# nyu-systems/Grendel-GS

Measured on AMD Instinct MI355X. Metric: training iters/sec (fwd+bwd), higher is better.
Workload: dtype f32

## Files before the change

grendel-gs_amd/csrc/binning_persist.h:

```cpp
#pragma once

namespace {

constexpr int TT_SHIFT = 20;
constexpr uint32_t TT_MASK = (1u << TT_SHIFT) - 1u;
constexpr uint32_t GB_ABORT = 0x80000000u;
constexpr int GB_FAN = 32;
constexpr int GB_LEAF_STRIDE = 32;
constexpr uint32_t PAIRS_ABORTED = 0xFFFFFFFFu;

struct GridSync {
    uint32_t *leaf;
    uint32_t *root;
    uint32_t *flags;
};
__host__ __device__ inline size_t grid_sync_words(int G) {
    return (size_t)(2 * ((G + GB_FAN - 1) / GB_FAN) + 1) * GB_LEAF_STRIDE;
}

__device__ __forceinline__ bool grid_barrier_try_abort(const GridSync gs, uint32_t complete) {
    uint32_t r = __hip_atomic_load(gs.root, __ATOMIC_RELAXED, __HIP_MEMORY_SCOPE_AGENT);
    while (true) {
        if (r & GB_ABORT) return true;
        if (r == complete) return false;
// ... 232 lines not shown
    out.ys = (uint32_t)miny | ((uint32_t)maxy << 16);
    out.mask = ~0ull;
    if (!cull || w * h > 64) {
        if (dxy) {
            atomicAdd(&dxy[0][minx], h);
            atomicAdd(&dxy[0][maxx], -h);
            atomicAdd(&dxy[1][miny], w);
            atomicAdd(&dxy[1][maxy], -w);
            atomicAdd(&dxy[2][miny], 1);
            atomicAdd(&dxy[2][maxy], -1);
        }
        return (uint32_t)(w * h);
    }
    const unsigned long long mask = gsr_tile_mask(xy, co, minx, miny, maxx, maxy);
    out.mask = mask;
    if (dxy) {
        const unsigned long long rowm = gsr_full_mask(w);
        int prev_cnt = 0, run_a0 = 0, run_len = 0, run_mult = 0;
        for (int r = 0; r < h; r++) {
            unsigned long long bits = (mask >> (r * w)) & rowm;
            const int cnt = __popcll(bits);
            if (cnt != prev_cnt) atomicAdd(&dxy[1][miny + r], cnt - prev_cnt);
            prev_cnt = cnt;
            while (bits) {
                const int a0 = __ffsll((long long)bits) - 1;
                const unsigned long long rest = ~(bits >> a0);
                const int len = rest ? __ffsll((long long)rest) - 1 : 64 - a0;
                if (run_mult && a0 == run_a0 && len == run_len) {
                    run_mult++;
                } else {
                    if (run_mult) {
                        atomicAdd(&dxy[0][minx + run_a0], run_mult);
                        atomicAdd(&dxy[0][minx + run_a0 + run_len], -run_mult);
                    }
                    run_a0 = a0; run_len = len; run_mult = 1;
                }
                bits &= ~(gsr_full_mask(len) << a0);
            }
        }
        if (run_mult) {
            atomicAdd(&dxy[0][minx + run_a0], run_mult);
            atomicAdd(&dxy[0][minx + run_a0 + run_len], -run_mult);
        }
        if (prev_cnt) atomicAdd(&dxy[1][maxy], -prev_cnt);
    }
    return (uint32_t)__popcll(mask);
}

template <int ITEMS, int THREADS>
struct PersistSmem {
    uint16_t wtab[THREADS / 64][RADIX_DIGITS];
    uint32_t gbase[RADIX_DIGITS];
    unsigned long long scan64[THREADS / 64];
    uint32_t scan_tmp[THREADS / 64];
    uint32_t flag;
    uint32_t skey[ITEMS * THREADS], sval[ITEMS * THREADS];
};

template <int ITEMS, int THREADS>
__device__ __forceinline__ void clear_wtab(PersistSmem<ITEMS, THREADS> &sm) {
    uint32_t *p = reinterpret_cast<uint32_t *>(&sm.wtab[0][0]);
    for (int i = threadIdx.x; i < (THREADS / 64) * RADIX_DIGITS / 2; i += THREADS) p[i] = 0u;
}

struct ByteDigit {
    int shift;
    uint32_t mask;
    __device__ __forceinline__ uint32_t operator()(uint32_t k) const { return (k >> shift) & mask; }
};
constexpr int BK_BINS = 4096, BK_BIN_BITS = 12;
constexpr uint32_t BK_TAIL = 255u;
struct BucketDigit {
    const uint8_t *map;
    uint32_t kmin;
    int sh;
    __device__ __forceinline__ uint32_t operator()(uint32_t k) const {
        return k == 0xFFFFFFFFu ? BK_TAIL : (uint32_t)map[(k - kmin) >> sh];
    }
};

template <int ITEMS, int THREADS, class DG>
__device__ __forceinline__ void count_wave_digits(PersistSmem<ITEMS, THREADS> &sm, const uint32_t (&key)[ITEMS],
                                                  long long wbase, long long n, const DG digit) {
    const int lane = threadIdx.x & 63, wave = threadIdx.x >> 6;
#pragma unroll
    for (int r = 0; r < ITEMS; r++) {
        if (wbase + r * 64 + lane < n) {
            const uint32_t dg = digit(key[r]);
            atomicAdd(reinterpret_cast<uint32_t *>(sm.wtab[wave]) + (dg >> 1), 1u << (16 * (dg & 1u)));
        }
    }
}
template <int ITEMS, int THREADS>
__device__ __forceinline__ void count_wave_digits(PersistSmem<ITEMS, THREADS> &sm, const uint32_t (&key)[ITEMS],
                                                  long long wbase, long long n, int shift, uint32_t mask) {
    count_wave_digits(sm, key, wbase, n, ByteDigit{shift, mask});
}

template <int ITEMS, int THREADS, class DG>
__device__ __forceinline__ void scatter_rank(PersistSmem<ITEMS, THREADS> &sm, const uint32_t (&key)[ITEMS],
                                             const uint32_t (&val)[ITEMS], long long tbase, long long n, const DG digit,
                                             int nbits, uint32_t &tot_out, uint32_t &run_out) {
    constexpr int WAVES = THREADS / 64;
    const int lane = threadIdx.x & 63, wave = threadIdx.x >> 6;
    const long long wbase = tbase + (long long)wave * (ITEMS * 64);
    const uint32_t d = threadIdx.x;
    uint32_t cnt[WAVES], tot = 0;
#pragma unroll
    for (int w = 0; w < WAVES; w++) {
        cnt[w] = d < RADIX_DIGITS ? sm.wtab[w][d] : 0u;
        tot += cnt[w];
    }
    uint32_t all;
    uint32_t run = block_exclusive_scan_n<WAVES>(tot, sm.scan_tmp, &all);
    tot_out = tot;
    run_out = run;
    if (d < RADIX_DIGITS) {
#pragma unroll
        for (int w = 0; w < WAVES; w++) {
            sm.wtab[w][d] = (uint16_t)run;
            run += cnt[w];
        }
    }
    __syncthreads();
    const unsigned long long lt = (1ull << lane) - 1ull;
#pragma unroll
    for (int r = 0; r < ITEMS; r++) {
        const bool valid = wbase + r * 64 + lane < n;
        const uint32_t dg = digit(key[r]);
        const unsigned long long m = match_digit(dg, valid, nbits);
        const uint32_t rank = __popcll(m & lt);
        uint16_t *cursor = sm.wtab[wave];
        uint32_t pos = 0;
        if (valid) pos = cursor[dg] + rank;
        asm volatile("" ::: "memory");
        __builtin_amdgcn_wave_barrier();
        if (valid && rank == 0) cursor[dg] = (uint16_t)(pos + (uint32_t)__popcll(m));
        asm volatile("" ::: "memory");
        __builtin_amdgcn_wave_barrier();
        if (valid) {
            sm.skey[pos] = key[r];
            sm.sval[pos] = val[r];
        }
    }
}

template <int ITEMS, int THREADS>
__device__ __forceinline__ void scatter_rank(PersistSmem<ITEMS, THREADS> &sm, const uint32_t (&key)[ITEMS],
                                             const uint32_t (&val)[ITEMS], long long tbase, long long n, int shift,
                                             int nbits, uint32_t &tot_out, uint32_t &run_out) {
    scatter_rank(sm, key, val, tbase, n, ByteDigit{shift, (1u << nbits) - 1u}, nbits, tot_out, run_out);
}

template <int ITEMS, int THREADS, bool WT_VALS>
__device__ __forceinline__ void scatter_write(PersistSmem<ITEMS, THREADS> &sm, long long tbase, long long n, int shift,
                                              int nbits, uint32_t first, uint32_t run, uint32_t *__restrict__ keys_out,
                                              uint32_t *__restrict__ vals_out) {
    constexpr int TILE = ITEMS * THREADS;
    const uint32_t mask = (1u << nbits) - 1u;
    if (threadIdx.x < RADIX_DIGITS) sm.gbase[threadIdx.x] = first - run;
    __syncthreads();
    const long long rem = n - tbase;
    const int count = rem < TILE ? (int)rem : TILE;
#pragma unroll
    for (int r = 0; r < ITEMS; r++) {
        const int i = r * THREADS + threadIdx.x;
        if (i < count) {
            const uint32_t k = sm.skey[i];
            const uint32_t dst = sm.gbase[(k >> shift) & mask] + (uint32_t)i;
            st_agent(&keys_out[dst], k);
            if (WT_VALS) st_agent(&vals_out[dst], sm.sval[i]);
            else vals_out[dst] = sm.sval[i];
        }
    }
    __syncthreads();
}

template <int ITEMS, int THREADS, bool WT_VALS>
__device__ __forceinline__ uint32_t scatter_tile(PersistSmem<ITEMS, THREADS> &sm, const uint32_t (&key)[ITEMS],
                                                 const uint32_t (&val)[ITEMS], long long tbase, long long n, int shift,
                                                 int nbits, uint32_t first, uint32_t *__restrict__ keys_out,
                                                 uint32_t *__restrict__ vals_out) {
    uint32_t tot, run;
    scatter_rank(sm, key, val, tbase, n, shift, nbits, tot, run);
    scatter_write<ITEMS, THREADS, WT_VALS>(sm, tbase, n, shift, nbits, first, run, keys_out, vals_out);
    return tot;
}

__device__ __forceinline__ unsigned long long wave_sum64(unsigned long long v) {
#pragma unroll
    for (int d = 32; d >= 1; d >>= 1) v += __shfl_xor(v, d, 64);
    return v;
}

__device__ __forceinline__ uint32_t xor_lane(uint32_t v, int lane, int d) {
    return (uint32_t)__builtin_amdgcn_ds_bpermute((lane ^ d) << 2, (int)v);
}
__device__ __forceinline__ int opaque_lane() {
    int lane = threadIdx.x & 63;
    asm volatile("" : "+v"(lane));
    return lane;
}
__device__ __forceinline__ unsigned long long wave_sum64_local(unsigned long long v) {
    const int lane = opaque_lane();
#pragma unroll
    for (int d = 32; d >= 1; d >>= 1)
        v += (unsigned long long)xor_lane((uint32_t)v, lane, d) | ((unsigned long long)xor_lane((uint32_t)(v >> 32), lane, d) << 32);
    return v;
}

__device__ __forceinline__ uint32_t clamp_pair_count(unsigned long long d) {
    return d >= 0xFFFFFFFEull ? 0xFFFFFFFEu : (uint32_t)d;
}
__device__ __forceinline__ void publish_pair_count(unsigned long long *early, unsigned long long mine, uint32_t nwg,
                                                   uint32_t *host_total, uint32_t seq) {
    __hip_atomic_fetch_add(early, mine, __ATOMIC_RELAXED, __HIP_MEMORY_SCOPE_AGENT);
    uint32_t *ticket = reinterpret_cast<uint32_t *>(early + 1);
    const uint32_t t = __hip_atomic_fetch_add(ticket, 1u, __ATOMIC_ACQ_REL, __HIP_MEMORY_SCOPE_AGENT);
    if (t + 1u == nwg && host_total) {
        const unsigned long long d = __hip_atomic_load(early, __ATOMIC_RELAXED, __HIP_MEMORY_SCOPE_AGENT);
        __hip_atomic_store(host_total, clamp_pair_count(d), __ATOMIC_RELAXED, __HIP_MEMORY_SCOPE_SYSTEM);
        __hip_atomic_store(host_total + 1, seq, __ATOMIC_RELEASE, __HIP_MEMORY_SCOPE_SYSTEM);
    }
}

#define GSR_TS(k)                                                                                       \
    do {                                                                                                \
        if (a.tstamp && threadIdx.x == 0) a.tstamp[(size_t)blockIdx.x * 32 + (k)] = __builtin_amdgcn_s_memrealtime(); \
    } while (0)

constexpr int PP_THREADS = 1024, PP_WAVES = PP_THREADS / 64;
constexpr int PP_MAX_TPW = 8;

struct PrepPersistArgs {
    int P, gx, gy;
    const float2 *means2D;
    const float *depths;
    const int32_t *radii;
    const float4 *conic_opacity;
    const uint8_t *mask;
    uint32_t *tt, *kA, *vA, *kB, *vB, *offsets;
    uint32_t *segoff;
    TileRect *rects;
    uint32_t *tile_hist;
    int cull;
    int32_t *hull_out;
    unsigned long long *early;
    uint4 *zero16;
    size_t zero16_n;
    GridSync sync;
    uint32_t *cnt;
    uint32_t *grp;
    unsigned long long *wtot;
    uint32_t *bins;
    int depth_buckets;
    uint32_t *host_total;
    uint32_t seq;
    uint32_t *done_word;
    uint32_t done_seq;
    uint64_t timeout_ticks;
    int force_abort;
    unsigned long long *tstamp;
};

struct PPExtra {
    int32_t dxy[3][RADIX_DIGITS + 1];
    int s_lo, s_hi;
};

constexpr int BK_ITEMS = 8;
constexpr int BK_CAP = BK_ITEMS * PP_THREADS;
constexpr int BK_PASS = RADIX_MAX_PASSES;
struct PPBucket {
    uint8_t map[BK_BINS];
    uint32_t lo, n, live;
};

template <int ITEMS, int THREADS>
__device__ __forceinline__ void bucket_scatter_write(PersistSmem<ITEMS, THREADS> &sm, long long n, const BucketDigit digit,
                                                     uint32_t first, uint32_t run, uint32_t *__restrict__ keys_out,
                                                     uint32_t *__restrict__ vals_out, uint32_t *__restrict__ ids_out) {
    constexpr int TILE = ITEMS * THREADS;
    if (threadIdx.x < RADIX_DIGITS) sm.gbase[threadIdx.x] = first - run;
    __syncthreads();
    const int count = n < TILE ? (int)n : TILE;
#pragma unroll
    for (int r = 0; r < ITEMS; r++) {
        const int i = r * THREADS + threadIdx.x;
        if (i < count) {
            const uint32_t k = sm.skey[i];
            const uint32_t dg = digit(k);
            const uint32_t dst = sm.gbase[dg] + (uint32_t)i;
            if (dg == BK_TAIL) {
                ids_out[dst] = sm.sval[i];
            } else {
                st_agent(&keys_out[dst], k);
                st_agent(&vals_out[dst], sm.sval[i]);
            }
        }
    }
    __syncthreads();
}

template <int THREADS>
__device__ __forceinline__ void bucket_sort_span(PersistSmem<BK_ITEMS, THREADS> &s, const uint32_t *__restrict__ kin,
                                                 const uint32_t *__restrict__ vin, uint32_t lo, uint32_t n,
                                                 uint32_t *__restrict__ red) {
    constexpr int WAVES = THREADS / 64;
    const int lane = threadIdx.x & 63, wave = threadIdx.x >> 6;
    const uint32_t wbase = (uint32_t)wave * (BK_ITEMS * 64);
    uint32_t key[BK_ITEMS], val[BK_ITEMS];
    uint32_t mn = 0xFFFFFFFFu, mx = 0u;
#pragma unroll
    for (int r = 0; r < BK_ITEMS; r++) {
        const uint32_t i = wbase + r * 64 + lane;
        key[r] = i < n ? ld_agent(&kin[lo + i]) : 0xFFFFFFFFu;
        val[r] = i < n ? ld_agent(&vin[lo + i]) : 0u;
    }
#pragma unroll
    for (int r = 0; r < BK_ITEMS; r++) {
        if (wbase + r * 64 + lane < n) {
            mn = min(mn, key[r]);
            mx = max(mx, key[r]);
        }
    }
#pragma unroll
    for (int d = 32; d >= 1; d >>= 1) {
        mn = min(mn, (uint32_t)__shfl_xor(mn, d, 64));
        mx = max(mx, (uint32_t)__shfl_xor(mx, d, 64));
    }
    if (lane == 0) {
        red[wave] = mn;
        red[WAVES + wave] = mx;
    }
    __syncthreads();
#pragma unroll
    for (int wv = 0; wv < WAVES; wv++) {
        mn = min(mn, red[wv]);
        mx = max(mx, red[WAVES + wv]);
    }
    const uint32_t diff = mx > mn ? mx - mn : 0u;
    const int nbits = diff ? 32 - __clz(diff) : 0;
#pragma unroll
    for (int r = 0; r < BK_ITEMS; r++) key[r] -= mn;
    if (nbits == 0) {
#pragma unroll
        for (int r = 0; r < BK_ITEMS; r++) {
            const uint32_t i = wbase + r * 64 + lane;
            if (i < n) s.sval[i] = val[r];
        }
        __syncthreads();
        return;
    }
    const int passes = (nbits + 7) / 8, pb = (nbits + passes - 1) / passes;
    for (int shift = 0; shift < nbits; shift += pb) {
        clear_wtab(s);
        __syncthreads();
        count_wave_digits(s, key, (long long)wbase, (long long)n, shift, (1u << pb) - 1u);
        __syncthreads();
        uint32_t tot, run;
        scatter_rank(s, key, val, 0ll, (long long)n, shift, pb, tot, run);
        __syncthreads();
        if (shift + pb < nbits) {
#pragma unroll
            for (int r = 0; r < BK_ITEMS; r++) {
                const uint32_t i = wbase + r * 64 + lane;
                if (i < n) {
                    key[r] = s.skey[i];
                    val[r] = s.sval[i];
                }
            }
            __syncthreads();
        }
    }
}


template <int PP_ITEMS>
__global__ void __launch_bounds__(PP_THREADS)
bin_prepare_persist_kernel(const PrepPersistArgs a) {
    constexpr int PP_TILE = PP_THREADS * PP_ITEMS;
    __shared__ PersistSmem<BK_ITEMS, PP_THREADS> sm8;
    PersistSmem<PP_ITEMS, PP_THREADS> &sm = *reinterpret_cast<PersistSmem<PP_ITEMS, PP_THREADS> *>(&sm8);
    __shared__ PPExtra ex;
    __shared__ PPBucket bk;
    __shared__ uint32_t red2[2 * PP_THREADS];
    const uint32_t G = gridDim.x, w = blockIdx.x;
    const int lane = threadIdx.x & 63, wave = threadIdx.x >> 6;
    const long long P = a.P;
    const long long nb = (P + PP_TILE - 1) / PP_TILE;
    const long long t0 = (long long)w * nb / G, t1 = (long long)(w + 1) * nb / G;
    const bool keep = (t1 - t0) == 1;
    const bool try_buckets = a.depth_buckets && nb == (long long)G && counts_fit_registers<PP_THREADS>(G);
    const uint32_t d = threadIdx.x;
    uint32_t epoch = 0;
    GSR_TS(0);
    uint32_t key[PP_ITEMS], val[PP_ITEMS];
    for (size_t i = (size_t)w * PP_THREADS + threadIdx.x; i < a.zero16_n; i += (size_t)G * PP_THREADS)
        a.zero16[i] = make_uint4(0u, 0u, 0u, 0u);

    if (threadIdx.x <= RADIX_DIGITS) ex.dxy[0][threadIdx.x] = ex.dxy[1][threadIdx.x] = ex.dxy[2][threadIdx.x] = 0;
    if (threadIdx.x == 0) { ex.s_lo = a.gy; ex.s_hi = 0; }
    clear_wtab(sm);
    __syncthreads();
    {
        const int total = a.gx * a.gy;
        const int per = (total + PP_THREADS - 1) / PP_THREADS;
        const int b0 = threadIdx.x * per, b1 = min(b0 + per, total);
        int first = 0x7fffffff, last = -1;
#pragma unroll 8
        for (int b = b0; b < b1; b++) {
            const int on = a.mask[b] != 0;
            first = min(first, on ? b : 0x7fffffff);
            last = max(last, on ? b : -1);
        }
        if (last >= 0) {
            atomicMin(&ex.s_lo, first / a.gx);
            atomicMax(&ex.s_hi, last / a.gx + 1);
        }
    }
    __syncthreads();
    const int hull0 = ex.s_lo, hull1 = ex.s_hi;
    if (w == 0 && threadIdx.x == 0) {
        a.hull_out[0] = hull1 > hull0 ? hull0 : 0;
        a.hull_out[1] = hull1 > hull0 ? hull1 : 0;
    }
    uint32_t mytot = 0;
    unsigned long long nsum = 0;
    uint32_t kmn = 0xFFFFFFFFu, kmx = 0u;
    for (long long t = t0; t < t1; t++) {
        const long long wbase = t * PP_TILE + (long long)wave * (PP_ITEMS * 64);
#pragma unroll
        for (int r0 = 0; r0 < PP_ITEMS; r0 += 4) {
        int rad[4];
        float2 xy[4];
        float4 co[4];
        float dep[4];
#pragma unroll
        for (int q4 = 0; q4 < 4; q4++) {
            const int r = r0 + q4;
            const long long i = wbase + r * 64 + lane;
            const long long ic = i < P ? i : P - 1;
            rad[q4] = a.radii[ic];
            xy[q4] = a.means2D[ic];
            co[q4] = a.conic_opacity[ic];
            dep[q4] = a.depths[ic];
        }
#pragma unroll
        for (int q4 = 0; q4 < 4; q4++) {
            const int r = r0 + q4;
            const long long i = wbase + r * 64 + lane;
            key[r] = 0xFFFFFFFFu;
            val[r] = (uint32_t)i;
            if (i < P) {
                uint32_t n = 0;
                TileRect rect{0u, 0u, 0ull};
                if (rad[q4] > 0) {
                    float exx, eyy;
                    if (gsr_alpha_extent(co[q4], exx, eyy)) {
                        int minx, miny, maxx, maxy;
                        gsr_get_rect(xy[q4].x, xy[q4].y, rad[q4], a.gx, a.gy, minx, miny, maxx, maxy);
                        miny = max(miny, hull0);
                        maxy = min(maxy, hull1);
                        gsr_narrow_span(xy[q4].x, exx, minx, maxx);
                        gsr_narrow_span(xy[q4].y, eyy, miny, maxy);
                        if (maxx > minx && maxy > miny)
                            n = gsr_rect_tiles(xy[q4], co[q4], minx, miny, maxx, maxy, a.cull != 0,
                                               a.tile_hist ? ex.dxy : nullptr, rect);
                    }
                }
                if (n) {
                    key[r] = __float_as_uint(dep[q4]);
                    kmn = min(kmn, key[r]);
                    kmx = max(kmx, key[r]);
                }
                nsum += n;
                st_agent(&a.tt[i], (a.tile_hist && n) ? (n | (((rect.ys >> 16) - (rect.ys & 0xFFFFu)) << TT_SHIFT)) : n);
                a.rects[i] = rect;
                if (!keep) {
                    st_agent(&a.kA[i], key[r]);
                    st_agent(&a.vA[i], val[r]);
                }
            }
        }
        }
        if (try_buckets) continue;
        count_wave_digits(sm, key, wbase, P, 0, 0xFFu);
        __syncthreads();
        if (d < RADIX_DIGITS) {
#pragma unroll
            for (int wv = 0; wv < PP_WAVES; wv++) mytot += sm.wtab[wv][d];
        }
        if (!keep) {
            __syncthreads();
            clear_wtab(sm);
            __syncthreads();
        }
    }
    if (!try_buckets && d < RADIX_DIGITS) publish_counts(a.cnt, a.grp, w, d, mytot);
    {
        nsum = wave_sum64_local(nsum);
        {
            const int ol = opaque_lane();
#pragma unroll
            for (int o = 32; o >= 1; o >>= 1) {
                kmn = min(kmn, xor_lane(kmn, ol, o));
                kmx = max(kmx, xor_lane(kmx, ol, o));
            }
        }
        __syncthreads();
        if (lane == 0) {
            sm.scan64[wave] = nsum;
            red2[wave] = kmn;
            red2[PP_WAVES + wave] = kmx;
        }
        __syncthreads();
        if (threadIdx.x == 0) {
            unsigned long long tot = 0;
            for (int wv = 0; wv < PP_WAVES; wv++) {
                tot += sm.scan64[wv];
                kmn = min(kmn, red2[wv]);
                kmx = max(kmx, red2[PP_WAVES + wv]);
            }
            if (tot) __hip_atomic_fetch_add(a.early, tot, __ATOMIC_RELAXED, __HIP_MEMORY_SCOPE_AGENT);
            if (try_buckets && kmn <= kmx) {
                __hip_atomic_fetch_max(&a.bins[BK_BINS], ~kmn, __ATOMIC_RELAXED, __HIP_MEMORY_SCOPE_AGENT);
                __hip_atomic_fetch_max(&a.bins[BK_BINS + 1], kmx, __ATOMIC_RELAXED, __HIP_MEMORY_SCOPE_AGENT);
            }
        }
    }
    if (a.tile_hist) {
        const uint32_t xcc = __builtin_amdgcn_s_getreg(20 | (3 << 11)) & 7u;
        for (int p = 0; p < 3; p++) {
            const uint32_t v = threadIdx.x < RADIX_DIGITS ? (uint32_t)ex.dxy[p][threadIdx.x] : 0u;
            uint32_t all;
            const uint32_t c = block_exclusive_scan_n<PP_WAVES>(v, sm.scan_tmp, &all) + v;
            if (threadIdx.x < RADIX_DIGITS && c)
                __hip_atomic_fetch_add(&a.tile_hist[(xcc * RADIX_MAX_PASSES + p) * RADIX_DIGITS + threadIdx.x], c,
                                       __ATOMIC_RELAXED, __HIP_MEMORY_SCOPE_WORKGROUP);
        }
    }
    GSR_TS(1);
    if (!grid_barrier(a.sync, G, epoch, a.timeout_ticks, &sm.flag, a.force_abort != 0)) {
        if (threadIdx.x == 0) {
            a.offsets[P] = PAIRS_ABORTED;
            __hip_atomic_store(a.host_total, PAIRS_ABORTED, __ATOMIC_RELAXED, __HIP_MEMORY_SCOPE_SYSTEM);
            __hip_atomic_store(a.host_total + 1, a.seq, __ATOMIC_RELEASE, __HIP_MEMORY_SCOPE_SYSTEM);
            if (a.done_seq) __hip_atomic_store(a.done_word, a.done_seq, __ATOMIC_RELEASE, __HIP_MEMORY_SCOPE_SYSTEM);
        }
        return;
    }
    GSR_TS(2);
    if (w == 0 && threadIdx.x == 0) {
        const unsigned long long dsum = __hip_atomic_load(a.early, __ATOMIC_RELAXED, __HIP_MEMORY_SCOPE_AGENT);
        __hip_atomic_store(a.host_total, clamp_pair_count(dsum), __ATOMIC_RELAXED, __HIP_MEMORY_SCOPE_SYSTEM);
        __hip_atomic_store(a.host_total + 1, a.seq, __ATOMIC_RELEASE, __HIP_MEMORY_SCOPE_SYSTEM);
    }
    const uint64_t forever = 100000000ull;
    const uint32_t ngroups = (G + GB_FAN - 1) / GB_FAN;
    if (try_buckets) {
        static_assert(BK_BINS == 4 * PP_THREADS, "four bins per thread");
        const long long wbase0 = t0 * PP_TILE + (long long)wave * (PP_ITEMS * 64);
        const uint32_t kmin = ~ld_agent(&a.bins[BK_BINS]), kmax = ld_agent(&a.bins[BK_BINS + 1]);
        const uint32_t NB = min(G, BK_TAIL);
        bool buckets = kmin <= kmax && kmax != 0xFFFFFFFFu;
        if (buckets) {
            const uint32_t range = kmax - kmin;
            const int sh = max((range ? 32 - __clz(range) : 0) - BK_BIN_BITS, 0);
            const BucketDigit digit{bk.map, kmin, sh};
            uint32_t *const lbin = sm8.skey;
            for (int i = threadIdx.x; i < BK_BINS; i += PP_THREADS) lbin[i] = 0u;
            __syncthreads();
#pragma unroll
            for (int r = 0; r < PP_ITEMS; r++)
                if (key[r] != 0xFFFFFFFFu) atomicAdd(&lbin[(key[r] - kmin) >> sh], 1u);
            __syncthreads();
            for (int i = threadIdx.x; i < BK_BINS; i += PP_THREADS) {
                const uint32_t c = lbin[i];
                if (c) __hip_atomic_fetch_add(&a.bins[i], c, __ATOMIC_RELAXED, __HIP_MEMORY_SCOPE_AGENT);
            }
            GSR_TS(21);
            if (!grid_barrier(a.sync, G, epoch, forever, &sm.flag)) { barrier_fault(a.done_word, 0x200u + epoch); return; }
            GSR_TS(22);
            {
                uint32_t c4[4], s4 = 0, live;
#pragma unroll
                for (int k = 0; k < 4; k++) {
                    c4[k] = ld_agent(&a.bins[threadIdx.x * 4 + k]);
                    s4 += c4[k];
                }
                uint32_t start = block_exclusive_scan_n<PP_WAVES>(s4, sm.scan_tmp, &live);
#pragma unroll
                for (int k = 0; k < 4; k++) {
                    bk.map[threadIdx.x * 4 + k] = (uint8_t)(start * NB / live);
                    start += c4[k];
                }
            }
            __syncthreads();
            count_wave_digits(sm, key, wbase0, P, digit);
            __syncthreads();
            if (d < RADIX_DIGITS) {
                mytot = 0;
#pragma unroll
                for (int wv = 0; wv < PP_WAVES; wv++) mytot += sm.wtab[wv][d];
                publish_counts(a.cnt + (size_t)BK_PASS * G * RADIX_DIGITS, a.grp + (size_t)BK_PASS * ngroups * RADIX_DIGITS, w,
                               d, mytot);
            }
            GSR_TS(23);
            if (!grid_barrier(a.sync, G, epoch, forever, &sm.flag)) { barrier_fault(a.done_word, 0x200u + epoch); return; }
            GSR_TS(24);
            uint32_t tot, run, before, total, all;
            counts_before<PP_THREADS>(a.cnt + (size_t)BK_PASS * G * RADIX_DIGITS,
                                      a.grp + (size_t)BK_PASS * ngroups * RADIX_DIGITS, G, w,
                                      reinterpret_cast<uint32_t *>(red2), before, total);
            if (__syncthreads_or(d < BK_TAIL && total > (uint32_t)BK_CAP)) {
                buckets = false;
            } else {
                scatter_rank(sm, key, val, t0 * PP_TILE, P, digit, 8, tot, run);
                const uint32_t dstart = block_exclusive_scan_n<PP_WAVES>(total, sm.scan_tmp, &all);
                if (d == w) {
                    bk.lo = dstart;
                    bk.n = w < NB ? total : 0u;
                }
                if (d == BK_TAIL) bk.live = dstart;
                bucket_scatter_write(sm, P - t0 * PP_TILE, digit, dstart + before, run, a.kB, a.vB, a.vA);
            }
        }
        if (buckets) {
            GSR_TS(25);
            if (!grid_barrier(a.sync, G, epoch, forever, &sm.flag)) { barrier_fault(a.done_word, 0x200u + epoch); return; }
            GSR_TS(26);
            const uint32_t lo = bk.lo, n = bk.n, live = bk.live;
            bucket_sort_span<PP_THREADS>(sm8, a.kB, a.vB, lo, n, reinterpret_cast<uint32_t *>(red2));
#pragma unroll
            for (int r = 0; r < BK_ITEMS; r++) {
                const uint32_t i = r * PP_THREADS + threadIdx.x;
                if (i < n) a.vA[lo + i] = sm8.sval[i];
            }
            uint32_t v[BK_ITEMS], hv[BK_ITEMS], s = 0, sh2 = 0;
#pragma unroll
            for (int k = 0; k < BK_ITEMS; k++) {
                const uint32_t i = threadIdx.x * BK_ITEMS + k;
                const uint32_t x = i < n ? ld_agent(&a.tt[sm8.sval[i]]) : 0u;
                v[k] = a.tile_hist ? (x & TT_MASK) : x;
                hv[k] = a.tile_hist ? (x >> TT_SHIFT) : 0u;
                s += v[k];
                sh2 += hv[k];
            }
            unsigned long long wsum = wave_sum64((unsigned long long)s | ((unsigned long long)sh2 << 32));
            if (lane == 0) sm.scan64[wave] = wsum;
            __syncthreads();
            if (threadIdx.x == 0) {
                unsigned long long tot = 0;
                for (int wv = 0; wv < PP_WAVES; wv++) tot += sm.scan64[wv];
                st_agent64(&a.wtot[w], tot);
            }
            GSR_TS(27);
            if (!grid_barrier(a.sync, G, epoch, forever, &sm.flag)) { barrier_fault(a.done_word, 0x200u + epoch); return; }
            GSR_TS(28);
            if (w == 0 && threadIdx.x == 0 && a.done_seq)
                __hip_atomic_store(a.done_word, a.done_seq, __ATOMIC_RELEASE, __HIP_MEMORY_SCOPE_SYSTEM);
            unsigned long long carry, gtot;
            {
                unsigned long long x = 0, y = 0;
                for (uint32_t k = threadIdx.x; k < G; k += PP_THREADS) {
                    const unsigned long long t = ld_agent64(&a.wtot[k]);
                    y += t;
                    if (k < w) x += t;
                }
                x = wave_sum64(x);
                y = wave_sum64(y);
                __syncthreads();
                if (lane == 0) {
                    sm.scan64[wave] = x;
                    reinterpret_cast<unsigned long long *>(red2)[wave] = y;
                }
                __syncthreads();
                carry = gtot = 0;
                for (int wv = 0; wv < PP_WAVES; wv++) {
                    carry += sm.scan64[wv];
                    gtot += reinterpret_cast<unsigned long long *>(red2)[wv];
                }
            }
            uint32_t tots, toth;
            const uint32_t local = block_exclusive_scan_n<PP_WAVES>(s, sm.scan_tmp, &tots);
            const uint32_t localh = block_exclusive_scan_n<PP_WAVES>(sh2, sm.scan_tmp, &toth);
            uint32_t runp = (uint32_t)carry + local, runh = (uint32_t)(carry >> 32) + localh;
#pragma unroll
            for (int k = 0; k < BK_ITEMS; k++) {
                const uint32_t i = threadIdx.x * BK_ITEMS + k;
                if (i < n) {
                    a.offsets[lo + i] = runp;
                    a.segoff[lo + i] = runh;
                }
                runp += v[k];
                runh += hv[k];
            }
            for (long long j = (long long)live + (long long)w * PP_THREADS + threadIdx.x; j < P; j += (long long)G * PP_THREADS) {
                a.offsets[j] = (uint32_t)gtot;
                a.segoff[j] = (uint32_t)(gtot >> 32);
            }
            if (w == G - 1 && threadIdx.x == 0) {
                a.offsets[P] = clamp_pair_count(__hip_atomic_load(a.early, __ATOMIC_RELAXED, __HIP_MEMORY_SCOPE_AGENT));
                a.segoff[P] = (uint32_t)(gtot >> 32);
            }
            GSR_TS(31);
            return;
        }
        __syncthreads();
        clear_wtab(sm);
        __syncthreads();
        count_wave_digits(sm, key, wbase0, P, 0, 0xFFu);
        __syncthreads();
        if (d < RADIX_DIGITS) {
            mytot = 0;
#pragma unroll
            for (int wv = 0; wv < PP_WAVES; wv++) mytot += sm.wtab[wv][d];
            publish_counts(a.cnt, a.grp, w, d, mytot);
        }
        GSR_TS(17);
        if (!grid_barrier(a.sync, G, epoch, forever, &sm.flag)) { barrier_fault(a.done_word, 0x200u + epoch); return; }
        GSR_TS(18);
    }
    for (int p = 0; p < 4; p++) {
        const int shift = 8 * p;
        uint32_t *const ksrc = (p & 1) ? a.kB : a.kA, *const vsrc = (p & 1) ? a.vB : a.vA;
        uint32_t *const kdst = (p & 1) ? a.kA : a.kB, *const vdst = (p & 1) ? a.vA : a.vB;
        const uint32_t *const cnt_p = a.cnt + (size_t)p * G * RADIX_DIGITS;
        const uint32_t *const grp_p = a.grp + (size_t)p * ngroups * RADIX_DIGITS;
        uint32_t before, total, all, first;
        if (keep && counts_fit_registers<PP_THREADS>(G)) {
            uint32_t wp = w;
            asm volatile("" : "+s"(wp));
            CountLoads cl;
            counts_issue<PP_THREADS>(cnt_p, grp_p, G, wp, cl);
            uint32_t tot, run;
            scatter_rank(sm, key, val, t0 * PP_TILE, P, shift, 8, tot, run);
            counts_finish<PP_THREADS>(cl, wp, reinterpret_cast<uint32_t *>(red2), before, total);
            first = block_exclusive_scan_n<PP_WAVES>(total, sm.scan_tmp, &all) + before;
            scatter_write<PP_ITEMS, PP_THREADS, true>(sm, t0 * PP_TILE, P, shift, 8, first, run, kdst, vdst);
        } else {
        counts_before<PP_THREADS>(cnt_p, grp_p, G, w, sm.skey, before, total);
        first = block_exclusive_scan_n<PP_WAVES>(total, sm.scan_tmp, &all) + before;
        for (long long t = t0; t < t1; t++) {
            const long long tbase = t * PP_TILE;
            const long long wbase = tbase + (long long)wave * (PP_ITEMS * 64);
            if (!keep) {
#pragma unroll
                for (int r = 0; r < PP_ITEMS; r++) {
                    const long long j = wbase + r * 64 + lane;
                    key[r] = j < P ? ld_agent(&ksrc[j]) : 0xFFFFFFFFu;
                    val[r] = j < P ? ld_agent(&vsrc[j]) : 0u;
                }
                count_wave_digits(sm, key, wbase, P, shift, 0xFFu);
                __syncthreads();
            }
            first += scatter_tile<PP_ITEMS, PP_THREADS, true>(sm, key, val, tbase, P, shift, 8, first, kdst, vdst);
            if (!keep) {
                clear_wtab(sm);
                __syncthreads();
            }
        }
        }
        GSR_TS(3 + 4 * p);
        if (!grid_barrier(a.sync, G, epoch, forever, &sm.flag)) { barrier_fault(a.done_word, 0x100u + epoch); return; }
        GSR_TS(4 + 4 * p);
        if (p == 3) break;
        if (keep) {
            clear_wtab(sm);
            __syncthreads();
        }
        mytot = 0;
        for (long long t = t0; t < t1; t++) {
            const long long wbase = t * PP_TILE + (long long)wave * (PP_ITEMS * 64);
#pragma unroll
            for (int r = 0; r < PP_ITEMS; r++) {
                const long long j = wbase + r * 64 + lane;
                key[r] = j < P ? ld_agent(&kdst[j]) : 0xFFFFFFFFu;
                val[r] = j < P ? ld_agent(&vdst[j]) : 0u;
            }
            count_wave_digits(sm, key, wbase, P, shift + 8, 0xFFu);
            __syncthreads();
            if (d < RADIX_DIGITS) {
#pragma unroll
                for (int wv = 0; wv < PP_WAVES; wv++) mytot += sm.wtab[wv][d];
            }
            if (!keep) {
                __syncthreads();
                clear_wtab(sm);
                __syncthreads();
            }
        }
        if (d < RADIX_DIGITS)
            publish_counts(a.cnt + (size_t)(p + 1) * G * RADIX_DIGITS, a.grp + (size_t)(p + 1) * ngroups * RADIX_DIGITS,
                           w, d, mytot);
        GSR_TS(5 + 4 * p);
        if (!grid_barrier(a.sync, G, epoch, forever, &sm.flag)) { barrier_fault(a.done_word, 0x100u + epoch); return; }
        GSR_TS(6 + 4 * p);
    }
    uint32_t v[PP_ITEMS], hv[PP_ITEMS];
    unsigned long long wsum = 0;
    for (long long t = t0; t < t1; t++) {
        const long long base = t * PP_TILE + (long long)threadIdx.x * PP_ITEMS;
        uint32_t s = 0, sh = 0;
#pragma unroll
        for (int k = 0; k < PP_ITEMS; k++) {
            const uint32_t x = (base + k < P) ? ld_agent(&a.tt[ld_agent(&a.vA[base + k])]) : 0u;
            v[k] = a.tile_hist ? (x & TT_MASK) : x;
            hv[k] = a.tile_hist ? (x >> TT_SHIFT) : 0u;
            s += v[k];
            sh += hv[k];
        }
        wsum += (unsigned long long)s | ((unsigned long long)sh << 32);
    }
    wsum = wave_sum64(wsum);
    if (lane == 0) sm.scan64[wave] = wsum;
    __syncthreads();
    if (threadIdx.x == 0) {
        unsigned long long tot = 0;
        for (int wv = 0; wv < PP_WAVES; wv++) tot += sm.scan64[wv];
        st_agent64(&a.wtot[w], tot);
    }
    GSR_TS(19);
    if (!grid_barrier(a.sync, G, epoch, forever, &sm.flag)) { barrier_fault(a.done_word, 0x100u + epoch); return; }
    GSR_TS(20);
    if (w == 0 && threadIdx.x == 0 && a.done_seq)
        __hip_atomic_store(a.done_word, a.done_seq, __ATOMIC_RELEASE, __HIP_MEMORY_SCOPE_SYSTEM);
    unsigned long long carry;
    {
        unsigned long long x = 0;
        for (uint32_t k = threadIdx.x; k < w; k += PP_THREADS) x += ld_agent64(&a.wtot[k]);
        x = wave_sum64(x);
        __syncthreads();
        if (lane == 0) sm.scan64[wave] = x;
        __syncthreads();
        carry = 0;
        for (int wv = 0; wv < PP_WAVES; wv++) carry += sm.scan64[wv];
    }
    for (long long t = t0; t < t1; t++) {
        const long long base = t * PP_TILE + (long long)threadIdx.x * PP_ITEMS;
        uint32_t s = 0, sh = 0;
        if (!keep) {
#pragma unroll
            for (int k = 0; k < PP_ITEMS; k++) {
                const uint32_t x = (base + k < P) ? ld_agent(&a.tt[ld_agent(&a.vA[base + k])]) : 0u;
                v[k] = a.tile_hist ? (x & TT_MASK) : x;
                hv[k] = a.tile_hist ? (x >> TT_SHIFT) : 0u;
            }
        }
#pragma unroll
        for (int k = 0; k < PP_ITEMS; k++) {
            s += v[k];
            sh += hv[k];
        }
        uint32_t tot, toth;
        const uint32_t local = block_exclusive_scan_n<PP_WAVES>(s, sm.scan_tmp, &tot);
        const uint32_t localh = block_exclusive_scan_n<PP_WAVES>(sh, sm.scan_tmp, &toth);
        uint32_t run = (uint32_t)carry + local, runh = (uint32_t)(carry >> 32) + localh;
#pragma unroll
        for (int k = 0; k < PP_ITEMS; k++) {
            if (base + k < P) {
                a.offsets[base + k] = run;
                a.segoff[base + k] = runh;
            }
            run += v[k];
            runh += hv[k];
        }
        carry += (unsigned long long)tot | ((unsigned long long)toth << 32);
    }
    if (w == G - 1 && threadIdx.x == 0) {
        a.offsets[P] = clamp_pair_count(__hip_atomic_load(a.early, __ATOMIC_RELAXED, __HIP_MEMORY_SCOPE_AGENT));
        a.segoff[P] = (uint32_t)(carry >> 32);
    }
    GSR_TS(31);
}

constexpr int PS_THREADS = 512, PS_ITEMS = 8, PS_TILE = PS_THREADS * PS_ITEMS, PS_WAVES = PS_THREADS / 64;
constexpr int PS_CHUNK = PS_ITEMS * 64;
#ifndef GSR_PS_DECODE_BATCH
#define GSR_PS_DECODE_BATCH 4
#endif
#ifndef GSR_PS_MIN_WAVES
#define GSR_PS_MIN_WAVES 4
#endif
constexpr int PS_MIN_WAVES = GSR_PS_MIN_WAVES;
constexpr int PS_OWNERS = 256;
static_assert(PS_TILE == RADIX_TILE, "tiles of both pipelines have 4096 elements");

struct SortPersistArgs {
    int P, gx, xbits, ybits;
    long long D;
    int bounded;
    const TileRect *rects;
    const uint32_t *sorted_ids;
    const uint32_t *offsets;
    const uint8_t *mask;
    uint32_t *kA, *kB, *vB, *point_list;
    int32_t *ranges;
    int ranges_words;
    const int32_t *hull;
    GridSync sync;
    uint32_t *cnt;
    uint32_t *grp;
    uint32_t *cnt_solo, *grp_solo;
    uint32_t *done_word;
    uint32_t done_seq;
    uint64_t timeout_ticks;
    int owners_cap;
    int force_abort;
    unsigned long long *tstamp;
};

struct PSExtra {
    int32_t dcol[RADIX_DIGITS + 1];
    int32_t owner[PS_OWNERS];
    uint32_t cflag[PS_WAVES][PS_CHUNK / 32];
    int j0, j1;
};

__device__ __forceinline__ int owner_search(const uint32_t *__restrict__ offsets, int lo, int hi, uint32_t s) {
    const int lane = threadIdx.x & 63;
    while (hi - lo > 1) {
        const int step = (hi - lo + 63) / 64;
        const int idx = min(lo + lane * step, hi);
        const bool le = offsets[idx] <= s;
        const int c = __popcll(__ballot(le));
        const int nlo = lo + (c - 1) * step;
        hi = min(hi, nlo + step);
        lo = nlo;
    }
    return lo;
}

template <int BATCH>
__device__ __forceinline__ void decode_chunk(const uint32_t *__restrict__ offsets, const uint32_t *__restrict__ sorted_ids,
                                             const TileRect *__restrict__ rects, int P, long long D, long long wbase, int g0,
// ... 318 lines not shown
```

Measured before the change: 853.6.

## Use wider 10-bit radix passes with peer-mask ranking in bucket local sort

Replaces the 8-bit-per-pass local radix sort inside each bucket with up to 10-bit passes, using packed 16-bit per-wave digit counters and a shared-memory peer-bitmask scheme to rank equal digits within a wave. Fewer passes mean fewer shared-memory scatter rounds and block barriers for wide key ranges. It adds a separate shared table (more LDS, possibly lower occupancy), atomics on packed counters, and optional timestamp probes; the old path is kept behind an ablation macro.

Result: no change. 858.7, median of 6 (+0.6%).

```diff
diff --git a/grendel-gs_amd/csrc/binning_persist.h b/grendel-gs_amd/csrc/binning_persist.h
--- a/grendel-gs_amd/csrc/binning_persist.h
+++ b/grendel-gs_amd/csrc/binning_persist.h
@@ -558,10 +558,85 @@
     __syncthreads();
 }
 
+constexpr int LS_BITS = 10, LS_PEER_BITS = 7;
 template <int THREADS>
-__device__ __forceinline__ void bucket_sort_span(PersistSmem<BK_ITEMS, THREADS> &s, const uint32_t *__restrict__ kin,
-                                                 const uint32_t *__restrict__ vin, uint32_t lo, uint32_t n,
-                                                 uint32_t *__restrict__ red) {
+struct LocalSortTab {
+    uint16_t tab[(THREADS / 64) << LS_BITS];
+    unsigned long long peers[THREADS / 64][1 << LS_PEER_BITS];
+};
+
+template <int THREADS>
+__device__ __forceinline__ void local_sort_pass(PersistSmem<BK_ITEMS, THREADS> &s, LocalSortTab<THREADS> &lt,
+                                                const uint32_t (&key)[BK_ITEMS], const uint32_t (&val)[BK_ITEMS],
+                                                uint32_t wbase, uint32_t n, int shift, int pb) {
+    constexpr int WAVES = THREADS / 64;
+    static_assert(THREADS >= (1 << LS_BITS), "one thread per digit in the scan");
+    const int lane = threadIdx.x & 63, wave = threadIdx.x >> 6;
+    const uint32_t mask = (1u << pb) - 1u, d = threadIdx.x;
+    uint32_t *const words = reinterpret_cast<uint32_t *>(lt.tab);
+    for (int i = threadIdx.x; i < (WAVES << pb) / 2; i += THREADS) words[i] = 0u;
+    __syncthreads();
+    uint16_t *const mine = lt.tab + ((uint32_t)wave << pb);
+#pragma unroll
+    for (int r = 0; r < BK_ITEMS; r++) {
+        if (wbase + r * 64 + lane < n) {
+            const uint32_t dg = (key[r] >> shift) & mask;
+            atomicAdd(reinterpret_cast<uint32_t *>(mine) + (dg >> 1), 1u << (16 * (dg & 1u)));
+        }
+    }
+    __syncthreads();
+    uint32_t cnt[WAVES], tot = 0;
+#pragma unroll
+    for (int w = 0; w < WAVES; w++) {
+        cnt[w] = d <= mask ? lt.tab[((uint32_t)w << pb) + d] : 0u;
+        tot += cnt[w];
+    }
+    uint32_t all;
+    uint32_t run = block_exclusive_scan_n<WAVES>(tot, s.scan_tmp, &all);
+    if (d <= mask) {
+#pragma unroll
+        for (int w = 0; w < WAVES; w++) {
+            lt.tab[((uint32_t)w << pb) + d] = (uint16_t)run;
+            run += cnt[w];
+        }
+    }
+    __syncthreads();
+    const unsigned long long below = (1ull << lane) - 1ull;
+    const int lb = pb > LS_PEER_BITS ? pb - LS_PEER_BITS : 0;
+    unsigned long long *const peers = lt.peers[wave];
+#pragma unroll
+    for (int r = 0; r < BK_ITEMS; r++) {
+        const bool valid = wbase + r * 64 + lane < n;
+        const uint32_t dg = (key[r] >> shift) & mask;
+        if (valid) atomicOr(&peers[dg >> lb], 1ull << lane);
+        asm volatile("" ::: "memory");
+        __builtin_amdgcn_wave_barrier();
+        unsigned long long m = valid ? peers[dg >> lb] : 0ull;
+        asm volatile("" ::: "memory");
+        __builtin_amdgcn_wave_barrier();
+        if (valid) peers[dg >> lb] = 0ull;
+        m &= match_digit(dg, valid, lb);
+        const uint32_t rank = __popcll(m & below);
+        uint32_t pos = 0;
+        if (valid) pos = mine[dg] + rank;
+        asm volatile("" ::: "memory");
+        __builtin_amdgcn_wave_barrier();
+        if (valid && rank == 0) mine[dg] = (uint16_t)(pos + (uint32_t)__popcll(m));
+        asm volatile("" ::: "memory");
+        __builtin_amdgcn_wave_barrier();
+        if (valid) {
+            s.skey[pos] = key[r];
+            s.sval[pos] = val[r];
+        }
+    }
+    __syncthreads();
+}
+
+template <int THREADS>
+__device__ __forceinline__ void bucket_sort_span(PersistSmem<BK_ITEMS, THREADS> &s, LocalSortTab<THREADS> &lt,
+                                                 const uint32_t *__restrict__ kin, const uint32_t *__restrict__ vin,
+                                                 uint32_t lo, uint32_t n, uint32_t *__restrict__ red,
+                                                 unsigned long long *__restrict__ ts) {
     constexpr int WAVES = THREADS / 64;
     const int lane = threadIdx.x & 63, wave = threadIdx.x >> 6;
     const uint32_t wbase = (uint32_t)wave * (BK_ITEMS * 64);
@@ -589,6 +664,9 @@
         red[wave] = mn;
         red[WAVES + wave] = mx;
     }
+#ifndef GSR_ABL_LOCAL_SORT_NARROW
+    for (int i = threadIdx.x; i < WAVES << LS_PEER_BITS; i += THREADS) (&lt.peers[0][0])[i] = 0ull;
+#endif
     __syncthreads();
 #pragma unroll
     for (int wv = 0; wv < WAVES; wv++) {
@@ -608,8 +686,27 @@
         __syncthreads();
         return;
     }
+    if (ts && threadIdx.x == 0) ts[29] = __builtin_amdgcn_s_memrealtime();
+#ifndef GSR_ABL_LOCAL_SORT_NARROW
+    const int passes = (nbits + LS_BITS - 1) / LS_BITS, pb = (nbits + passes - 1) / passes;
+    for (int shift = 0, k = 0; shift < nbits; shift += pb, k++) {
+        local_sort_pass(s, lt, key, val, wbase, n, shift, pb);
+        if (ts && threadIdx.x == 0) ts[3 + k] = __builtin_amdgcn_s_memrealtime();
+        if (shift + pb < nbits) {
+#pragma unroll
+            for (int r = 0; r < BK_ITEMS; r++) {
+                const uint32_t i = wbase + r * 64 + lane;
+                if (i < n) {
+                    key[r] = s.skey[i];
+                    val[r] = s.sval[i];
+                }
+            }
+            __syncthreads();
+        }
+    }
+#else
     const int passes = (nbits + 7) / 8, pb = (nbits + passes - 1) / passes;
-    for (int shift = 0; shift < nbits; shift += pb) {
+    for (int shift = 0, k = 0; shift < nbits; shift += pb, k++) {
         clear_wtab(s);
         __syncthreads();
         count_wave_digits(s, key, (long long)wbase, (long long)n, shift, (1u << pb) - 1u);
@@ -617,6 +714,7 @@
         uint32_t tot, run;
         scatter_rank(s, key, val, 0ll, (long long)n, shift, pb, tot, run);
         __syncthreads();
+        if (ts && threadIdx.x == 0) ts[3 + k] = __builtin_amdgcn_s_memrealtime();
         if (shift + pb < nbits) {
 #pragma unroll
             for (int r = 0; r < BK_ITEMS; r++) {
@@ -629,6 +727,7 @@
             __syncthreads();
         }
     }
+#endif
 }
 
 
@@ -641,6 +740,11 @@
     __shared__ PPExtra ex;
     __shared__ PPBucket bk;
     __shared__ uint32_t red2[2 * PP_THREADS];
+#ifndef GSR_ABL_LOCAL_SORT_NARROW
+    __shared__ LocalSortTab<PP_THREADS> lst;
+#else
+    LocalSortTab<PP_THREADS> &lst = *reinterpret_cast<LocalSortTab<PP_THREADS> *>(red2);
+#endif
     const uint32_t G = gridDim.x, w = blockIdx.x;
     const int lane = threadIdx.x & 63, wave = threadIdx.x >> 6;
     const long long P = a.P;
@@ -887,7 +991,8 @@
             if (!grid_barrier(a.sync, G, epoch, forever, &sm.flag)) { barrier_fault(a.done_word, 0x200u + epoch); return; }
             GSR_TS(26);
             const uint32_t lo = bk.lo, n = bk.n, live = bk.live;
-            bucket_sort_span<PP_THREADS>(sm8, a.kB, a.vB, lo, n, reinterpret_cast<uint32_t *>(red2));
+            bucket_sort_span<PP_THREADS>(sm8, lst, a.kB, a.vB, lo, n, reinterpret_cast<uint32_t *>(red2),
+                                         a.tstamp ? a.tstamp + (size_t)blockIdx.x * 32 : nullptr);
 #pragma unroll
             for (int r = 0; r < BK_ITEMS; r++) {
                 const uint32_t i = r * PP_THREADS + threadIdx.x;
```
